# NKI-CCB/bcm3

Hardware: AMD Instinct MI355X
Metric: log-likelihood evals/sec (whole node), PopPK ODE @256 chains; HBM-roofline % (higher is better)
Workload: dtype f64

## Files before the change

### bcm3_amd/csrc/host/SamplerPTDevice.cpp

```cpp
#include "SamplerPTDevice.h"

#include <algorithm>
#include <cmath>
#include <condition_variable>
#include <cstring>
#include <deque>
#include <limits>
#include <map>
#include <mutex>
#include <thread>

#include "../../../include/bcm3.h"
#include "../../../include/bcm3hip.h"
#include "GMM.h"
#include "NetCDFClassic.h"
#include "log.h"

namespace bcm3 {

static const double kInf = std::numeric_limits<double>::infinity();


static uint64_t SplitMix64(uint64_t x)
{
// ... 151 lines not shown
    std::shared_ptr<LocalGroup> g_;
    int rank_;
};

}

std::unique_ptr<Transport> MakeLocalTransport(std::shared_ptr<LocalGroup> group, int rank)
{
    if (!group || rank < 0 || rank >= group->world) return nullptr;
    return std::unique_ptr<Transport>(new LocalTransport(std::move(group), rank));
}


namespace {

template <class T>
struct DevBuf {
    T* p = nullptr;
    size_t n = 0;
    bool alloc(size_t count)
    {
        n = count;
        return bcm3hip_malloc((void**)&p, std::max<size_t>(count, 1) * sizeof(T)) == 0;
    }
    ~DevBuf() { bcm3hip_free(p); }
};

template <class T>
bool Upload(DevBuf<T>& b, const std::vector<T>& h, void* s)
{
    return bcm3hip_memcpy_async(b.p, h.data(), h.size() * sizeof(T), BCM3HIP_H2D, s) == 0;
}
template <class T>
bool Download(std::vector<T>& h, const DevBuf<T>& b, void* s)
{
    h.resize(b.n);
    return bcm3hip_memcpy_async(h.data(), b.p, b.n * sizeof(T), BCM3HIP_D2H, s) == 0 && bcm3hip_stream_synchronize(s) == 0;
}

}

struct SamplerPTDevice::Impl {
    PTMHConfig cfg;
    std::shared_ptr<Likelihood> ll;
    std::unique_ptr<Transport> transport;
    void* stream = nullptr;
    bool own_stream = false;
    int64_t C = 0, Ctot = 0, g0 = 0;
    int d = 0, kmax = 1, H = 1, sub = 1;
    bool adaptive = true, adjusted = false;
    int kind = 1;
    std::vector<double> temps_host, prior_mean, prior_var;
    double target = 0.234;

    DevBuf<int32_t> pkind;
    DevBuf<double> p0, p1, p2, lower, upper, rw_scale, temps, zeros;
    DevBuf<double> values, prop, lprior, lprior_prop, llh, llh_prop, lpp, log_mh;
    DevBuf<int32_t> status, nan_flag;
    DevBuf<uint64_t> acc_mutate, acc_exchange;
    DevBuf<int32_t> ncomp, selected;
    DevBuf<double> weights, mean, chol, logc, scale, ema, work;
    bcm3hip_proposal P{};
    DevBuf<float> hist;
    DevBuf<int64_t> hcount;
    std::vector<std::unique_ptr<DevBuf<uint8_t>>> masks[2];
    bool mask_all[2] = {false, false};
    DevBuf<uint8_t> pair_mask;
    DevBuf<double> send_last, send_first, recv_next, recv_prev;

    PTMHCounters cnt;
    int64_t iter = 0, round = 0;

    bool blocked = false;
    int max_blocks = 1;
    std::vector<int32_t> bl_n, bl_off, bl_vars;
    std::vector<int64_t> sub_decisions;
    DevBuf<int32_t> b_nblocks, b_offset, b_vars, b_ncomp, b_selected;
    DevBuf<double> b_target, b_weights, b_logc, b_scale, b_ema, b_mean, b_chol;
    DevBuf<uint8_t> b_active;
    bcm3hip_blocks B{};

    bool spec_on = false;
    bool spec_tail_on = true;
    DevBuf<double> sp_cand_x, sp_cand_lp, sp_cand_lmh, sp_cand_llh, sp_cand_sc, sp_batch_x, sp_batch_llh;
    DevBuf<int32_t> sp_cand_sel, sp_cand_upd, sp_cand_steps, sp_steps_hint, sp_steps_prop, sp_batch_status,
        sp_batch_steps, sp_batch_src, sp_batch_n, sp_err;
    DevBuf<int32_t> sp_pos;
    DevBuf<float> sp_xs;
    DevBuf<int64_t> sp_total;
    DevBuf<uint8_t> sp_cand_active, acc_mut, acc_mut2, acc_exc;
    DevBuf<int32_t> partner[2], pair_first[2];
    DevBuf<double> sp_send_last, sp_send_first, sp_remote;
    DevBuf<uint8_t> cross_acc;
    DevBuf<int32_t> sp_pred;
    DevBuf<double> sp_inv_scale;
    bool cross_round[2] = {false, false};
    bcm3hip_spec S{};
    int64_t spec_pairs = 0;
    int spec_first_round = 0;

    std::unique_ptr<SampleFileWriter> out;
    DevBuf<double> out_buf;
    bool out_on = false, out_gather = false;
    DevBuf<double> out_recv;
    int64_t out_samples = 0, out_first = 0, out_pending = 0, emitted = 0;
    int out_flush = 64;
    bool out_overflow_logged = false;
    std::string adapt_file;
    BundleFile adapt_out;

    bool Emit()
    {
        const int64_t six = emitted++;
        if (!out_on) return true;
        if (six >= out_samples) {
            if (!out_overflow_logged) LOGWARNING("More samples than the output file holds (%lld); later samples are not stored", (long long)out_samples);
            out_overflow_logged = true;
            return true;
        }
        if (out_pending == 0) out_first = six;
        double* slot = out_buf.p + out_pending * C * (d + 2);
        if (bcm3hip_memcpy_async(slot, values.p, C * d * sizeof(double), BCM3HIP_D2D, stream) != 0 ||
            bcm3hip_memcpy_async(slot + C * d, lprior.p, C * sizeof(double), BCM3HIP_D2D, stream) != 0 ||
            bcm3hip_memcpy_async(slot + C * (d + 1), llh.p, C * sizeof(double), BCM3HIP_D2D, stream) != 0)
            return false;
        out_pending++;
        if (out_pending == out_flush || six + 1 == out_samples) return Flush();
        return true;
    }

    bool Flush()
    {
        if (!out_on || out_pending == 0) return true;
        if (out_gather) return FlushGather();
        std::vector<double> h((size_t)(out_pending * C * (d + 2)));
        if (bcm3hip_memcpy_async(h.data(), out_buf.p, h.size() * sizeof(double), BCM3HIP_D2H, stream) != 0 ||
            bcm3hip_stream_synchronize(stream) != 0)
            return false;
        const std::vector<double> w(C, 1.0);
        for (int64_t k = 0; k < out_pending; k++) {
            const double* r = &h[(size_t)(k * C * (d + 2))];
            if (!out->Write((size_t)(out_first + k), 0, (size_t)C, r, r + C * d, r + C * (d + 1), w.data())) {
                LOGERROR("Writing sample %lld to the output file failed", (long long)(out_first + k));
                return false;
            }
        }
        out_pending = 0;
        return true;
    }

    bool FlushGather()
    {
        const size_t cnt = (size_t)(out_pending * C * (d + 2));
        const int world = cfg.world, rank = cfg.rank;
        if (rank != 0) {
            const double* sp = out_buf.p;
            const int peer = 0;
            if (!transport || !transport->Exchange(1, &sp, &peer, 0, nullptr, nullptr, cnt, stream)) {
                LOGERROR("Sending sample rows to rank 0 failed (rank %d)", rank);
                return false;
            }
            out_pending = 0;
            return bcm3hip_stream_synchronize(stream) == 0;
        }
        std::vector<double*> recvs((size_t)(world - 1));
        std::vector<int> peers((size_t)(world - 1));
// ... 391 lines not shown
            speer[ns++] = Prev();
            recvs[nr] = recv_prev.p;
            rpeer[nr++] = Prev();
        }
        if (do_next) {
            recvs[nr] = recv_next.p;
            rpeer[nr++] = Next();
        }
        if (!transport || !transport->Exchange(ns, sends, speer, nr, recvs, rpeer, n, stream)) {
            LOGERROR("PT swap transport failed (rank %d)", cfg.rank);
            return false;
        }
        return Launch(bcm3hip_pt_cross_accept((int)C, d, g0, gp, do_next, do_prev, temps.p, values.p, llh.p,
                                              lprior.p, lpp.p, recv_next.p, recv_prev.p, acc_out,
                                              do_next ? acc_exchange.p : nullptr, cfg.seed, (uint64_t)round, stream),
                      "pt_cross_accept");
    }

    bool Exchange(uint8_t* acc_mask = nullptr, uint8_t* cross_out = nullptr)
    {
        if (Ctot < 2) return true;
        const int start = (int)(round % 2);
        const bool wrap_local = cfg.world == 1 && (Ctot - 1 - start) % 2 == 0;
        if (!Launch(bcm3hip_pt_exchange_local((int)C, d, g0, start, wrap_local ? 1 : 0, temps.p, values.p, llh.p,
                                              lprior.p, lpp.p, acc_mask, acc_exchange.p, cfg.seed, (uint64_t)round,
                                              stream),
                    "pt_exchange_local"))
            return false;
        int64_t attempted = wrap_local ? 1 : 0;
        for (int64_t i = 0; i + 1 < C; i++)
            if (((g0 + i - start) % 2 + 2) % 2 == 0) attempted++;
        if (cfg.world > 1 && ((g0 + C - 1 - start) % 2 + 2) % 2 == 0) {
            if (!Cross(true, true, (int64_t)Prev() * C + C - 1, cross_out)) return false;
            attempted++;
        }
        cnt.attempted_exchange += attempted;
        if (adaptive) {
            if (mask_all[start]) {
                if (!HistoryAdd(nullptr)) return false;
            } else {
                for (auto& m : masks[start])
                    if (!HistoryAdd(m->p)) return false;
            }
        }
        round++;
        return true;
    }

    bool ExchangeRandom()
    {
        const int64_t ci = RandomPair(cfg.seed, (uint64_t)round, Ctot);
        const int64_t l1 = ci - g0, l2 = ci + 1 - g0;
        if (0 <= l1 && l2 < C) {
            if (!Launch(bcm3hip_pt_exchange_pair((int)C, d, (int)l1, (int)l2, ci, temps.p, values.p, llh.p, lprior.p,
                                                 lpp.p, nullptr, acc_exchange.p, cfg.seed, (uint64_t)round, stream),
                        "pt_exchange_pair"))
                return false;
            cnt.attempted_exchange++;
        } else if (cfg.world > 1 && (l1 == C - 1 || l2 == 0)) {
            if (l1 == C - 1) {
                if (!Cross(true, false, 0)) return false;
                cnt.attempted_exchange++;
            } else if (!Cross(false, true, ci)) {
                return false;
            }
        }
        if (adaptive) {
            std::vector<uint8_t> m(C, 0);
            bool any = false;
            for (int64_t i : {l1, l2})
                if (0 <= i && i < C) {
                    m[i] = 1;
                    any = true;
                }
            if (any && (!Upload(pair_mask, m, stream) || !HistoryAdd(pair_mask.p))) return false;
        }
        round++;
        return true;
    }

    bool IterationOnce(bool last)
    {
        bool ok;
        if (Ctot < 2) {
            ok = Mutate();
        } else if (cfg.swapping_scheme == 0) {
            ok = Exchange();
            for (int s = 0; ok && s < cfg.exploration_steps; s++) ok = Mutate();
        } else if (MoveUniform(cfg.seed, (uint64_t)cnt.samples_done) < cfg.exchange_probability) {
            ok = (cfg.swapping_scheme == 1) ? Exchange() : ExchangeRandom();
        } else {
            ok = Mutate();
        }
        return ok && PostIteration(last);
    }

    bool AdaptDue(int64_t si, bool last) const
    {
        if (!adaptive || (si + 1) % cfg.use_every_nth != 0) return false;
        const int64_t sample_ix = si / cfg.use_every_nth;
        return cfg.adapt_proposal_samples > 0 && (sample_ix + 1) % cfg.adapt_proposal_samples == 0 && !last &&
               cnt.adaptations_done < cfg.adapt_proposal_times;
    }

    bool PostIteration(bool last)
    {
        const int64_t si = cnt.samples_done++;
        cnt.iterations++;
        if ((si + 1) % cfg.use_every_nth == 0 && !Emit()) return false;
        if (AdaptDue(si, last)) return Adapt();
        return true;
    }

    bool PairPossible() const { return spec_on && !AdaptDue(cnt.samples_done, false); }

    bool PairExchange()
    {
        const int st = (int)(round % 2);
        if (cfg.world == 1 && mask_all[st] && Ctot >= 2) {
            const bool wrap_local = (Ctot - 1 - st) % 2 == 0;
            int64_t attempted = wrap_local ? 1 : 0;
            for (int64_t i = 0; i + 1 < C; i++)
                if (((g0 + i - st) % 2 + 2) % 2 == 0) attempted++;
            if (!Launch(bcm3hip_ptmh_spec_exchange((int)C, d, g0, st, wrap_local ? 1 : 0, temps.p, values.p, llh.p,
                                                   lprior.p, lpp.p, acc_exc.p, acc_exchange.p, cfg.seed,
                                                   (uint64_t)round, partner[st].p, pair_first[st].p, &S, H, sub,
                                                   adaptive ? hist.p : nullptr, hcount.p, stream),
                        "ptmh_spec_exchange"))
                return false;
            cnt.attempted_exchange += attempted;
            round++;
            return true;
        }
        return Exchange(acc_exc.p, cross_acc.p) &&
               Launch(bcm3hip_ptmh_spec_track((int)C, nullptr, partner[st].p, pair_first[st].p, acc_exc.p, &S, stream),
                      "ptmh_spec_track");
    }

    bool TailFusable() const
    {
        const int st = (int)(round % 2);
        return cfg.world == 1 && mask_all[st] && Ctot >= 2 && C <= 4096 && S.batch_pos &&
               !(out_on && (cnt.samples_done + 1) % cfg.use_every_nth == 0) && spec_tail_on;
    }

    bool IterationPair(bool last)
    {
        if (!PairExchange()) return false;
        const int nxt = (int)(round % 2);
        if (!Launch(bcm3hip_ptmh_propose_adaptive((int)C, d, pkind.p, p0.p, p1.p, p2.p, temps.p, values.p, prop.p,
                                                  lprior_prop.p, log_mh.p, &P, g0, cfg.seed, (uint64_t)iter, stream),
                    "ptmh_propose_adaptive"))
            return false;
        if (cross_round[nxt]) {
            const size_t row = (size_t)d * sizeof(double);
            if (bcm3hip_memcpy_async(sp_send_last.p, values.p + (C - 1) * d, row, BCM3HIP_D2D, stream) != 0 ||
                bcm3hip_memcpy_async(sp_send_last.p + d, prop.p + (C - 1) * d, row, BCM3HIP_D2D, stream) != 0 ||
                bcm3hip_memcpy_async(sp_send_first.p, values.p, row, BCM3HIP_D2D, stream) != 0 ||
                bcm3hip_memcpy_async(sp_send_first.p + d, prop.p, row, BCM3HIP_D2D, stream) != 0)
                return false;
            const double* sends[2] = {sp_send_last.p, sp_send_first.p};
            const int speer[2] = {Next(), Prev()};
            double* recvs[2] = {sp_remote.p + 2 * d, sp_remote.p};
            const int rpeer[2] = {Prev(), Next()};
            if (!transport || !transport->Exchange(2, sends, speer, 2, recvs, rpeer, (size_t)(2 * d), stream)) {
                LOGERROR("speculative boundary rows: transport failed (rank %d)", cfg.rank);
                return false;
            }
        }
        if (!Launch(bcm3hip_ptmh_spec_candidates((int)C, d, pkind.p, p0.p, p1.p, p2.p, temps.p, values.p, prop.p,
                                                 partner[nxt].p, sp_remote.p, &P, &S, g0, cfg.seed, (uint64_t)iter + 1,
                                                 stream),
                    "ptmh_spec_candidates") ||
            !Launch(bcm3hip_ptmh_spec_batch((int)C, d, prop.p, partner[nxt].p, sp_inv_scale.p, spec_first_round, &S,
                                            stream),
                    "ptmh_spec_batch"))
            return false;
        cnt.likelihood_launches++;
        if (!ll->EvaluateLogProbabilityBatchDeviceCounted((size_t)C * (1 + BCM3HIP_SPEC_SLOTS), S.batch_n, S.batch_x,
                                                          S.batch_llh, S.batch_status, S.batch_steps, stream)) {
            LOGERROR("EvaluateLogProbabilityBatchDeviceCounted failed");
            return false;
        }
        if (TailFusable()) {
            const int st = (int)(round % 2);
            const bool wrap_local = (Ctot - 1 - st) % 2 == 0;
            int64_t attempted = wrap_local ? 1 : 0;
            for (int64_t i = 0; i + 1 < C; i++)
                if (((g0 + i - st) % 2 + 2) % 2 == 0) attempted++;
            if (!Launch(bcm3hip_ptmh_spec_tail((int)C, d, g0, st, wrap_local ? 1 : 0, temps.p, partner[st].p,
                                               pair_first[st].p, acc_mut.p, acc_mut2.p, acc_exc.p, cross_acc.p,
                                               sp_remote.p, acc_mutate.p, acc_exchange.p, &S, prop.p, lprior_prop.p,
                                               log_mh.p, llh_prop.p, cfg.learning_rate, values.p, lprior.p, llh.p, lpp.p,
                                               nan_flag.p, &P, cfg.seed, (uint64_t)iter, (uint64_t)round, H, sub, hist.p,
                                               hcount.p, sp_err.p, stream),
                        "ptmh_spec_tail"))
                return false;
            cnt.attempted_mutate += C;
            iter++;
            if (!PostIteration(false)) return false;
            cnt.attempted_exchange += attempted;
            round++;
            cnt.attempted_mutate += C;
            iter++;
            spec_pairs++;
            return PostIteration(last);
        }
        if (!Launch(bcm3hip_ptmh_spec_commit((int)C, d, 0, temps.p, nullptr, nullptr, nullptr, nullptr, nullptr, nullptr,
                                             &S, prop.p, lprior_prop.p, log_mh.p, llh_prop.p, cfg.learning_rate,
                                             values.p, lprior.p, llh.p, lpp.p, acc_mut.p, acc_mutate.p, nan_flag.p, &P,
                                             g0, cfg.seed, (uint64_t)iter, H, sub, hist.p, hcount.p, sp_err.p, stream),
                    "ptmh_spec_commit"))
            return false;
        cnt.attempted_mutate += C;
        iter++;
        if (!PostIteration(false)) return false;
        if (!PairExchange()) return false;
        if (!Launch(bcm3hip_ptmh_spec_commit((int)C, d, 1, temps.p, partner[nxt].p, pair_first[nxt].p, acc_mut.p,
                                             acc_exc.p, cross_acc.p, sp_remote.p, &S, prop.p, lprior_prop.p, log_mh.p,
                                             llh_prop.p, cfg.learning_rate, values.p, lprior.p, llh.p, lpp.p, acc_mut2.p,
                                             acc_mutate.p, nan_flag.p, &P, g0, cfg.seed, (uint64_t)iter, H, sub, hist.p,
                                             hcount.p, sp_err.p, stream),
                    "ptmh_spec_commit"))
            return false;
        cnt.attempted_mutate += C;
        iter++;
        spec_pairs++;
        return PostIteration(last);
    }

    bool Iterations(int64_t n, bool last_at_end, int64_t nan_every)
    {
        int64_t since_check = 0;
        for (int64_t i = 0; i < n;) {
            int64_t k;
            if (i + 2 <= n && PairPossible()) {
                if (!IterationPair(last_at_end && i + 2 == n)) return false;
                k = 2;
            } else {
                if (!IterationOnce(last_at_end && i + 1 == n)) return false;
                k = 1;
            }
            i += k;
            since_check += k;
            if (nan_every > 0 && since_check >= nan_every) {
                since_check = 0;
                if (!CheckNaN()) return false;
            }
        }
        return true;
    }

    bool SetupSpeculation()
    {
        spec_tail_on = getenv("BCM3_NO_SPEC_TAIL") == nullptr;
        spec_on = cfg.speculate != 0 && !blocked && adaptive && (cfg.world == 1 || transport) && cfg.swapping_scheme == 0 &&
                  cfg.exploration_steps == 1 && Ctot >= 2 && d <= 64 && C * (1 + BCM3HIP_SPEC_SLOTS) <= 4096 &&
                  ll->SupportsCountedBatch();
        if (!spec_on) return true;
        spec_first_round = bcm3hip_current_device_simds();
        const int64_t K = BCM3HIP_SPEC_SLOTS, N = C * (1 + K);
        bool ok = sp_cand_x.alloc(C * K * d) && sp_cand_lp.alloc(C * K) && sp_cand_lmh.alloc(C * K) &&
                  sp_cand_llh.alloc(C * K) && sp_cand_sc.alloc(C * K) && sp_cand_sel.alloc(C * K) &&
                  sp_cand_upd.alloc(C * K) && sp_cand_steps.alloc(C * K) && sp_cand_active.alloc(C * K) &&
                  sp_steps_hint.alloc(C) && sp_steps_prop.alloc(C) && sp_batch_x.alloc(N * d) &&
                  sp_batch_llh.alloc(N) && sp_batch_status.alloc(N) && sp_batch_steps.alloc(N) &&
                  sp_batch_src.alloc(N) && sp_batch_n.alloc(1) && sp_err.alloc(1) && acc_mut.alloc(C) &&
                  acc_mut2.alloc(C) &&
                  acc_exc.alloc(C) && sp_send_last.alloc(2 * d) && sp_send_first.alloc(2 * d) &&
                  sp_remote.alloc(4 * d) && cross_acc.alloc(2) && sp_pred.alloc(N) && sp_inv_scale.alloc(d) &&
                  sp_total.alloc(1) && sp_pos.alloc(N) && sp_xs.alloc(N * d);
        for (int st = 0; st < 2 && ok; st++) ok = partner[st].alloc(C) && pair_first[st].alloc(C);
        if (!ok) {
            LOGERROR("SamplerPTDevice: speculative buffers could not be allocated");
            return false;
        }
        for (int st = 0; st < 2; st++) {
            std::vector<int32_t> pa(C, -1), pf(C, -1);
            const int par = (int)(((g0 - st) % 2 + 2) % 2);
            for (int64_t i = par; i + 1 < C; i += 2) {
                pa[i] = (int32_t)(i + 1);
                pa[i + 1] = (int32_t)i;
                pf[i] = pf[i + 1] = (int32_t)i;
            }
            if (cfg.world == 1 && (Ctot - 1 - st) % 2 == 0) {
                pa[C - 1] = 0;
                pa[0] = (int32_t)(C - 1);
                pf[C - 1] = pf[0] = (int32_t)(C - 1);
            }
            cross_round[st] = cfg.world > 1 && ((g0 + C - 1 - st) % 2 + 2) % 2 == 0;
            if (cross_round[st]) {
                pa[C - 1] = BCM3HIP_SPEC_REMOTE_NEXT;
                pa[0] = BCM3HIP_SPEC_REMOTE_PREV;
            }
            if (!Upload(partner[st], pa, stream) || !Upload(pair_first[st], pf, stream)) return false;
        }
        std::vector<double> isc(d);
        for (int j = 0; j < d; j++)
            isc[j] = (prior_var[j] > 0.0 && std::isfinite(prior_var[j])) ? 1.0 / std::sqrt(prior_var[j]) : 1.0;
        if (!Upload(sp_inv_scale, isc, stream) ||
            bcm3hip_memset_async(sp_batch_n.p, 0, sizeof(int32_t), stream) != 0 ||
            bcm3hip_memset_async(sp_steps_hint.p, 0, C * sizeof(int32_t), stream) != 0 ||
            bcm3hip_memset_async(sp_batch_steps.p, 0, N * sizeof(int32_t), stream) != 0 ||
            bcm3hip_memset_async(sp_cand_steps.p, 0, C * K * sizeof(int32_t), stream) != 0 ||
            bcm3hip_memset_async(sp_err.p, 0, sizeof(int32_t), stream) != 0 ||
            bcm3hip_memset_async(sp_total.p, 0, sizeof(int64_t), stream) != 0)
            return false;
        S.cand_x = sp_cand_x.p;
        S.cand_lp = sp_cand_lp.p;
        S.cand_lmh = sp_cand_lmh.p;
        S.cand_llh = sp_cand_llh.p;
        S.cand_sel = sp_cand_sel.p;
        S.cand_upd = sp_cand_upd.p;
        S.cand_sc = sp_cand_sc.p;
        S.cand_active = sp_cand_active.p;
        S.cand_steps = sp_cand_steps.p;
        S.steps_hint = sp_steps_hint.p;
        S.steps_prop = sp_steps_prop.p;
        S.batch_x = sp_batch_x.p;
        S.batch_llh = sp_batch_llh.p;
        S.batch_status = sp_batch_status.p;
        S.batch_steps = sp_batch_steps.p;
        S.batch_src = sp_batch_src.p;
        S.batch_n = sp_batch_n.p;
        S.pred_steps = sp_pred.p;
        S.batch_total = sp_total.p;
        S.batch_pos = sp_pos.p;
        S.batch_xs = sp_xs.p;
        return true;
    }

    bool CheckNaN()
    {
        std::vector<int32_t> f;
        if (!Download(f, nan_flag, stream)) return false;
        if (f[0] != 0) {
            LOGERROR("Likelihood evaluation returned NaN (Sampler::EvaluateLikelihood, fatal)");
            return false;
// ... 461 lines not shown
```

### bcm3_amd/csrc/proposal_kernels.hip

```cpp
#include <hip/hip_runtime.h>

#include <cmath>
#include <cstdint>

#include "../../include/bcm3hip.h"
#include "ctr_rng.h"
#include "prior_marginal.h"
#include "pt_exchange.h"

namespace bcm3hip {
namespace {

using rng::normal01;
using rng::rng_key;
using rng::u01;

__device__ double logsum2(double loga, double logb)
{
    if (logb > loga) {
        const double t = loga;
        loga = logb;
        logb = t;
    }
    if (loga == -INFINITY) return loga;
// ... 1296 lines not shown
                                        bcm3hip_proposal P, int64_t chain0, uint64_t seed, uint64_t iter, int H,
                                        int subsampling, float* __restrict__ hist, int64_t* __restrict__ counters,
                                        int32_t* __restrict__ error)
{
    const int c = blockIdx.x * blockDim.x + threadIdx.x;
    if (c >= C) return;
    commit_one(c, C, d, select, temps, partner, pair_first, acc_prev, acc_exc, cross_acc, remote, S, prop, lprior_prop,
               log_mh, llh_prop, learning_rate, values, lprior, llh, lpp, acc_out, accepted, nan_llh, P, chain0, seed,
               iter, H, subsampling, hist, counters, error);
}

__global__ void ptmh_spec_track_accept_kernel(int C, const uint8_t* __restrict__ acc, bcm3hip_spec S)
{
    const int c = blockIdx.x * blockDim.x + threadIdx.x;
    if (c >= C) return;
    if (acc[c]) S.steps_hint[c] = S.steps_prop[c];
}
__global__ void __launch_bounds__(1024) ptmh_spec_track_exchange_kernel(int C, const int32_t* __restrict__ partner,
                                                                        const int32_t* __restrict__ pair_first,
                                                                        const uint8_t* __restrict__ acc_exc,
                                                                        bcm3hip_spec S)
{
    int v[4];
    int n = 0;
    for (int c = threadIdx.x; c < C && n < 4; c += blockDim.x, n++) {
        const int p = partner[c];
        v[n] = (p >= 0 && acc_exc[pair_first[c]]) ? S.steps_hint[p] : S.steps_hint[c];
    }
    __syncthreads();
    n = 0;
    for (int c = threadIdx.x; c < C && n < 4; c += blockDim.x, n++) S.steps_hint[c] = v[n];
}

__device__ __forceinline__ void exchange_round(int C, int d, int64_t g0, int start, int wrap_local, const double* temps, double* values,
                               double* llh, double* lprior, double* lpp, uint8_t* acc_mask,
                               unsigned long long* accepted, uint64_t seed, uint64_t round,
                               const int32_t* __restrict__ partner, const int32_t* __restrict__ pair_first,
                               const bcm3hip_spec& S, int H, int subsampling, float* __restrict__ hist,
                               int64_t* __restrict__ counters)
{
    const int par = (int)(((g0 - start) % 2 + 2) % 2);
    for (int p = threadIdx.x;; p += blockDim.x) {
        const int i = par + 2 * p;
        if (i + 1 >= C) break;
        exchange_pair(d, i, i + 1, g0 + i, temps, values, llh, lprior, lpp, acc_mask, accepted, seed, round);
    }
    __syncthreads();
    if (wrap_local && threadIdx.x == 0)
        exchange_pair(d, C - 1, 0, g0 + C - 1, temps, values, llh, lprior, lpp, acc_mask, accepted, seed, round);
    __syncthreads();
    int v[4];
    int n = 0;
    for (int c = threadIdx.x; c < C && n < 4; c += blockDim.x, n++) {
        const int p = partner[c];
        v[n] = (p >= 0 && acc_mask[pair_first[c]]) ? S.steps_hint[p] : S.steps_hint[c];
    }
    __syncthreads();
    n = 0;
    for (int c = threadIdx.x; c < C && n < 4; c += blockDim.x, n++) {
        S.steps_hint[c] = v[n];
        if (hist) history_one(c, d, H, subsampling, temps, values, nullptr, hist, counters);
    }
}

__global__ void __launch_bounds__(1024) ptmh_spec_exchange_kernel(
    int C, int d, int64_t g0, int start, int wrap_local, const double* temps, double* values, double* llh,
    double* lprior, double* lpp, uint8_t* acc_mask, unsigned long long* accepted, uint64_t seed, uint64_t round,
    const int32_t* __restrict__ partner, const int32_t* __restrict__ pair_first, bcm3hip_spec S, int H,
    int subsampling, float* __restrict__ hist, int64_t* __restrict__ counters)
{
    exchange_round(C, d, g0, start, wrap_local, temps, values, llh, lprior, lpp, acc_mask, accepted, seed, round, partner,
                   pair_first, S, H, subsampling, hist, counters);
}

__global__ void __launch_bounds__(1024) ptmh_spec_tail_kernel(
    int C, int d, int64_t g0, int start, int wrap_local, const double* __restrict__ temps,
    const int32_t* __restrict__ partner, const int32_t* __restrict__ pair_first, uint8_t* __restrict__ acc_mut,
    uint8_t* __restrict__ acc_mut2, uint8_t* __restrict__ acc_exc, const uint8_t* __restrict__ cross_acc,
    const double* __restrict__ remote, unsigned long long* __restrict__ acc_mutate,
    unsigned long long* __restrict__ acc_exchange, bcm3hip_spec S, double* __restrict__ prop,
    double* __restrict__ lprior_prop, double* __restrict__ log_mh, double* __restrict__ llh_prop, double learning_rate,
    double* __restrict__ values, double* __restrict__ lprior, double* __restrict__ llh, double* __restrict__ lpp,
    int32_t* __restrict__ nan_llh, bcm3hip_proposal P, uint64_t seed, uint64_t iter, uint64_t round, int H,
    int subsampling, float* __restrict__ hist, int64_t* __restrict__ counters, int32_t* __restrict__ error)
{
    for (int c = threadIdx.x; c < C; c += blockDim.x)
        commit_one(c, C, d, 0, temps, nullptr, nullptr, nullptr, nullptr, nullptr, nullptr, S, prop, lprior_prop, log_mh,
                   llh_prop, learning_rate, values, lprior, llh, lpp, acc_mut, acc_mutate, nan_llh, P, g0, seed, iter, H,
                   subsampling, hist, counters, error);
    __syncthreads();
    exchange_round(C, d, g0, start, wrap_local, temps, values, llh, lprior, lpp, acc_exc, acc_exchange, seed, round,
                   partner, pair_first, S, H, subsampling, hist, counters);
    __syncthreads();
    for (int c = threadIdx.x; c < C; c += blockDim.x)
        commit_one(c, C, d, 1, temps, partner, pair_first, acc_mut, acc_exc, cross_acc, remote, S, prop, lprior_prop,
                   log_mh, llh_prop, learning_rate, values, lprior, llh, lpp, acc_mut2, acc_mutate, nan_llh, P, g0, seed,
                   iter + 1, H, subsampling, hist, counters, error);
}

bool proposal_ok(const bcm3hip_proposal* P, int C, int d)
{
    if (!P || P->kmax < 1 || P->kmax > BCM3HIP_PROPOSAL_KMAX) return false;
    if (P->kind != BCM3HIP_PROPOSAL_GLOBAL_COVARIANCE && P->kind != BCM3HIP_PROPOSAL_GAUSSIAN_MIXTURE) return false;
    if (!(P->scaling_ema_period > 0.0) || !(P->t_dof >= 0.0)) return false;
    if (C > 0 && (!P->lower || !P->upper || !P->ncomp || !P->weights || !P->mean || !P->chol || !P->logc ||
                  !P->scale || !P->ema || !P->selected || !P->work))
        return false;
    return true;
}

}
}

using namespace bcm3hip;

extern "C" {

int bcm3hip_ptmh_propose_adaptive(int C, int d, const int32_t* prior_kind, const double* prior_p0,
                                  const double* prior_p1, const double* prior_p2, const double* temps,
                                  const double* values, double* prop, double* lprior_prop, double* log_mh,
                                  const bcm3hip_proposal* proposal, int64_t chain0, uint64_t seed, uint64_t iter,
                                  void* stream)
{
    if (C < 0 || d <= 0 || !proposal_ok(proposal, C, d) ||
        (C > 0 && (!prior_kind || !prior_p0 || !prior_p1 || !prior_p2 || !temps || !values || !prop ||
                   !lprior_prop || !log_mh)))
        return BCM3HIP_ERR_ARG;
    if (C == 0) return 0;
    if (d <= 64)
        hipLaunchKernelGGL(ptmh_propose_wave_kernel, dim3(C), dim3(64), 0, (hipStream_t)stream, C, d, prior_kind,
                           prior_p0, prior_p1, prior_p2, temps, values, prop, lprior_prop, log_mh, *proposal, chain0,
                           seed, iter);
    else
        hipLaunchKernelGGL(ptmh_propose_adaptive_kernel, dim3((C + 63) / 64), dim3(64), 0, (hipStream_t)stream, C,
                           d, prior_kind, prior_p0, prior_p1, prior_p2, temps, values, prop, lprior_prop, log_mh,
                           *proposal, chain0, seed, iter);
    return hipGetLastError() == hipSuccess ? 0 : BCM3HIP_ERR_HIP;
}

int bcm3hip_ptmh_accept_adaptive(int C, int d, const double* temps, const double* prop, const double* lprior_prop,
                                 const double* llh_prop, const double* log_mh, double learning_rate, double* values,
                                 double* lprior, double* llh, double* lpp, uint8_t* accept_out, uint64_t* accepted,
                                 int32_t* nan_llh, const bcm3hip_proposal* proposal, int64_t chain0, uint64_t seed,
                                 uint64_t iter, void* stream)
{
    if (C < 0 || d <= 0 || !proposal_ok(proposal, C, d) ||
        (C > 0 && (!temps || !prop || !lprior_prop || !llh_prop || !log_mh || !values || !lprior || !llh || !lpp)))
        return BCM3HIP_ERR_ARG;
    if (C == 0) return 0;
    hipLaunchKernelGGL(ptmh_accept_adaptive_kernel, dim3((C + 63) / 64), dim3(64), 0, (hipStream_t)stream, C, d,
                       temps, prop, lprior_prop, llh_prop, log_mh, learning_rate, values, lprior, llh, lpp, accept_out,
                       (unsigned long long*)accepted, nan_llh, *proposal, chain0, seed, iter);
    return hipGetLastError() == hipSuccess ? 0 : BCM3HIP_ERR_HIP;
}

static bool blocked_ok(const bcm3hip_proposal* P, const bcm3hip_blocks* B, int C, int d, int submove)
{
    if (!P || !B || d > BCM3HIP_BLOCKED_MAX_D || submove < 0 || submove >= d) return false;
    if (P->kind != BCM3HIP_PROPOSAL_GLOBAL_COVARIANCE && P->kind != BCM3HIP_PROPOSAL_GAUSSIAN_MIXTURE) return false;
    if (P->kmax < 1 || P->kmax > BCM3HIP_PROPOSAL_KMAX) return false;
    if (C > 0 && (!P->lower || !P->upper || !B->nblocks || !B->block_offset || !B->block_vars || !B->target ||
                  !B->ncomp || !B->selected || !B->weights || !B->logc || !B->scale || !B->ema || !B->mean ||
                  !B->chol || !B->active))
        return false;
    return true;
}

int bcm3hip_ptmh_propose_blocked(int C, int d, int submove, const int32_t* prior_kind, const double* prior_p0,
                                 const double* prior_p1, const double* prior_p2, const double* temps,
                                 const double* values, double* prop, double* lprior_prop, double* log_mh,
                                 const bcm3hip_proposal* proposal, const bcm3hip_blocks* blocks, int64_t chain0,
                                 uint64_t seed, uint64_t iter, void* stream)
{
    if (C < 0 || d <= 0 || !blocked_ok(proposal, blocks, C, d, submove) ||
        (C > 0 && (!prior_kind || !prior_p0 || !prior_p1 || !prior_p2 || !temps || !values || !prop ||
                   !lprior_prop || !log_mh)))
        return BCM3HIP_ERR_ARG;
    if (C == 0) return 0;
    if (d <= 64)
        hipLaunchKernelGGL(ptmh_propose_blocked_kernel, dim3(C), dim3(64), 0, (hipStream_t)stream, C, d, submove,
// ... 48 lines not shown

int bcm3hip_ptmh_spec_batch(int C, int d, const double* prop, const int32_t* partner, const double* inv_scale,
                            int first_round, const bcm3hip_spec* spec, void* stream)
{
    if (C <= 0 || d <= 0 || C * (1 + BCM3HIP_SPEC_SLOTS) > kSpecSortMax || !prop || !partner || !inv_scale ||
        first_round < 0 || !spec_ok(spec) || !spec->pred_steps)
        return BCM3HIP_ERR_ARG;
    hipLaunchKernelGGL(ptmh_spec_predict_kernel, dim3(C * (1 + BCM3HIP_SPEC_SLOTS)), dim3(64 * kKnnWaves), 0,
                       (hipStream_t)stream,
                       C, d, prop, partner, inv_scale, *spec);
    hipLaunchKernelGGL(ptmh_spec_batch_kernel, dim3(1), dim3(1024), 0, (hipStream_t)stream, C, d, prop, partner,
                       first_round, inv_scale, *spec);
    return hipGetLastError() == hipSuccess ? 0 : BCM3HIP_ERR_HIP;
}

int bcm3hip_ptmh_spec_scatter(int C, const bcm3hip_spec* spec, double* llh_prop, void* stream)
{
    if (C <= 0 || !spec_ok(spec) || !llh_prop) return BCM3HIP_ERR_ARG;
    const int n = C * (1 + BCM3HIP_SPEC_SLOTS);
    hipLaunchKernelGGL(ptmh_spec_scatter_kernel, dim3((n + 255) / 256), dim3(256), 0, (hipStream_t)stream, C, *spec,
                       llh_prop);
    return hipGetLastError() == hipSuccess ? 0 : BCM3HIP_ERR_HIP;
}

int bcm3hip_ptmh_spec_select(int C, int d, const double* temps, const int32_t* partner, const int32_t* pair_first,
                             const uint8_t* acc_mutate, const uint8_t* acc_exchange, const uint8_t* cross_acc,
                             const double* remote, const double* values, const bcm3hip_spec* spec, double* prop,
                             double* lprior_prop, double* log_mh, double* llh_prop, const bcm3hip_proposal* proposal,
                             int32_t* error, void* stream)
{
    if (C <= 0 || d <= 0 || !temps || !partner || !pair_first || !acc_mutate || !acc_exchange || !spec_ok(spec) ||
        !values || !prop || !lprior_prop || !log_mh || !llh_prop || !proposal_ok(proposal, C, d))
        return BCM3HIP_ERR_ARG;
    hipLaunchKernelGGL(ptmh_spec_select_kernel, dim3((C + 63) / 64), dim3(64), 0, (hipStream_t)stream, C, d, temps,
                       partner, pair_first, acc_mutate, acc_exchange, cross_acc, remote, values, *spec, prop,
                       lprior_prop, log_mh, llh_prop, *proposal, error);
    return hipGetLastError() == hipSuccess ? 0 : BCM3HIP_ERR_HIP;
}

int bcm3hip_ptmh_spec_commit(int C, int d, int select, const double* temps, const int32_t* partner,
                             const int32_t* pair_first, const uint8_t* acc_prev, const uint8_t* acc_exchange,
                             const uint8_t* cross_acc, const double* remote, const bcm3hip_spec* spec, double* prop,
                             double* lprior_prop, double* log_mh, double* llh_prop, double learning_rate, double* values,
                             double* lprior, double* llh, double* lpp, uint8_t* accept_out, uint64_t* accepted,
                             int32_t* nan_llh, const bcm3hip_proposal* proposal, int64_t chain0, uint64_t seed,
                             uint64_t iter, int H, int subsampling, float* history, int64_t* counters, int32_t* error,
                             void* stream)
{
    if (C <= 0 || d <= 0 || !spec_ok(spec) || !proposal_ok(proposal, C, d) || !temps || !prop || !lprior_prop ||
        !log_mh || !llh_prop || !values || !lprior || !llh || !lpp || !accept_out ||
        (select && (!partner || !pair_first || !acc_prev || !acc_exchange || acc_prev == accept_out)) ||
        (history && (H <= 0 || subsampling <= 0 || !counters)))
        return BCM3HIP_ERR_ARG;
    hipLaunchKernelGGL(ptmh_spec_commit_kernel, dim3((C + 63) / 64), dim3(64), 0, (hipStream_t)stream, C, d, select,
                       temps, partner, pair_first, acc_prev, acc_exchange, cross_acc, remote, *spec, prop, lprior_prop,
                       log_mh, llh_prop, learning_rate, values, lprior, llh, lpp, accept_out,
                       (unsigned long long*)accepted, nan_llh, *proposal, chain0, seed, iter, H, subsampling, history,
                       counters, error);
    return hipGetLastError() == hipSuccess ? 0 : BCM3HIP_ERR_HIP;
}

int bcm3hip_ptmh_spec_exchange(int C, int d, int64_t g0, int start, int wrap_local, const double* temps,
                               double* values, double* llh, double* lprior, double* lpp, uint8_t* acc_exchange,
                               uint64_t* accepted, uint64_t seed, uint64_t round, const int32_t* partner,
                               const int32_t* pair_first, const bcm3hip_spec* spec, int H, int subsampling,
                               float* history, int64_t* counters, void* stream)
{
    if (C < 2 || C > 4096 || d <= 0 || !temps || !values || !llh || !lprior || !lpp || !acc_exchange || !partner ||
        !pair_first || !spec_ok(spec) || (history && (H <= 0 || subsampling <= 0 || !counters)))
        return BCM3HIP_ERR_ARG;
    hipLaunchKernelGGL(ptmh_spec_exchange_kernel, dim3(1), dim3(1024), 0, (hipStream_t)stream, C, d, g0, start,
                       wrap_local, temps, values, llh, lprior, lpp, acc_exchange, (unsigned long long*)accepted, seed,
                       round, partner, pair_first, *spec, H, subsampling, history, counters);
    return hipGetLastError() == hipSuccess ? 0 : BCM3HIP_ERR_HIP;
}

int bcm3hip_ptmh_spec_tail(int C, int d, int64_t g0, int start, int wrap_local, const double* temps,
                           const int32_t* partner, const int32_t* pair_first, uint8_t* acc_mut, uint8_t* acc_mut2,
                           uint8_t* acc_exc, const uint8_t* cross_acc, const double* remote, uint64_t* accepted_mutate,
                           uint64_t* accepted_exchange, const bcm3hip_spec* spec, double* prop, double* lprior_prop,
                           double* log_mh, double* llh_prop, double learning_rate, double* values, double* lprior,
                           double* llh, double* lpp, int32_t* nan_llh, const bcm3hip_proposal* proposal, uint64_t seed,
                           uint64_t iter, uint64_t round, int H, int subsampling, float* history, int64_t* counters,
                           int32_t* error, void* stream)
{
    if (C < 2 || C > 4096 || d <= 0 || !spec_ok(spec) || !spec->batch_pos || !proposal_ok(proposal, C, d) || !temps ||
        !partner || !pair_first || !acc_mut || !acc_mut2 || acc_mut == acc_mut2 || !acc_exc || !prop || !lprior_prop ||
        !log_mh || !llh_prop || !values || !lprior || !llh || !lpp || (history && (H <= 0 || subsampling <= 0 || !counters)))
        return BCM3HIP_ERR_ARG;
    hipLaunchKernelGGL(ptmh_spec_tail_kernel, dim3(1), dim3(1024), 0, (hipStream_t)stream, C, d, g0, start, wrap_local,
                       temps, partner, pair_first, acc_mut, acc_mut2, acc_exc, cross_acc, remote,
                       (unsigned long long*)accepted_mutate, (unsigned long long*)accepted_exchange, *spec, prop,
                       lprior_prop, log_mh, llh_prop, learning_rate, values, lprior, llh, lpp, nan_llh, *proposal, seed,
                       iter, round, H, subsampling, history, counters, error);
    return hipGetLastError() == hipSuccess ? 0 : BCM3HIP_ERR_HIP;
}

int bcm3hip_ptmh_spec_track(int C, const uint8_t* acc_mutate, const int32_t* partner, const int32_t* pair_first,
                            const uint8_t* acc_exchange, const bcm3hip_spec* spec, void* stream)
{
    if (C <= 0 || C > 4096 || !spec_ok(spec) || (!acc_mutate && !acc_exchange) ||
        (acc_exchange && (!partner || !pair_first)))
        return BCM3HIP_ERR_ARG;
    if (acc_mutate)
        hipLaunchKernelGGL(ptmh_spec_track_accept_kernel, dim3((C + 255) / 256), dim3(256), 0, (hipStream_t)stream, C,
                           acc_mutate, *spec);
    else
        hipLaunchKernelGGL(ptmh_spec_track_exchange_kernel, dim3(1), dim3(1024), 0, (hipStream_t)stream, C, partner,
                           pair_first, acc_exchange, *spec);
    return hipGetLastError() == hipSuccess ? 0 : BCM3HIP_ERR_HIP;
}

int bcm3hip_gmm_eval(int n, int d, int K, const double* x, const double* mean, const double* chol, const double* logc,
                     const double* weights, double* logpdf, double* resp, void* stream)
{
    if (n < 0 || d <= 0 || d > 64 || K <= 0 || K > 64 || (n > 0 && (!x || !mean || !chol || !logc || !weights)))
        return BCM3HIP_ERR_ARG;
    if (n == 0) return 0;
    hipLaunchKernelGGL(gmm_eval_wave_kernel, dim3(n), dim3(64), 0, (hipStream_t)stream, n, d, K, x, mean, chol, logc,
                       weights, logpdf, resp);
    return hipGetLastError() == hipSuccess ? 0 : BCM3HIP_ERR_HIP;
}

int bcm3hip_history_add(int C, int d, int H, int subsampling, const double* temps, const double* values,
                        const uint8_t* mask, float* history, int64_t* counters, void* stream)
{
    if (C < 0 || d <= 0 || H <= 0 || subsampling <= 0 || (C > 0 && (!temps || !values || !history || !counters)))
        return BCM3HIP_ERR_ARG;
    if (C == 0) return 0;
    hipLaunchKernelGGL(history_add_kernel, dim3((C + 63) / 64), dim3(64), 0, (hipStream_t)stream, C, d, H,
                       subsampling, temps, values, mask, history, counters);
    return hipGetLastError() == hipSuccess ? 0 : BCM3HIP_ERR_HIP;
}

}
```

### include/bcm3hip.h

```cpp
#ifndef BCM3HIP_H
#define BCM3HIP_H

#if !defined(__HIPCC_RTC__)
#include <stddef.h>
#include <stdint.h>
#endif

#ifdef __cplusplus
extern "C" {
#endif

#define BCM3HIP_OK 0
#define BCM3HIP_ERR_ARG (-1)
#define BCM3HIP_ERR_HIP (-2)
#define BCM3HIP_ERR_NODEVICE (-3)
#define BCM3HIP_ERR_MODEL (-4)
#define BCM3HIP_ERR_ALLOC (-5)

#define BCM3HIP_STATUS_OK 0
#define BCM3HIP_STATUS_SOLVER_FAIL 1

enum {
    BCM3HIP_PK_ONE = 0,
    BCM3HIP_PK_TWO = 1,
// ... 356 lines not shown
    const int32_t* nblocks;
    const int32_t* block_offset;
    const int32_t* block_vars;
    const double* target;
    int32_t* ncomp;
    int32_t* selected;
    double* weights;
    double* logc;
    double* scale;
    double* ema;
    double* mean;
    double* chol;
    uint8_t* active;
} bcm3hip_blocks;
int bcm3hip_ptmh_propose_blocked(int C, int d, int submove, const int32_t* prior_kind, const double* prior_p0,
                                 const double* prior_p1, const double* prior_p2, const double* temps,
                                 const double* values, double* prop, double* lprior_prop, double* log_mh,
                                 const bcm3hip_proposal* proposal, const bcm3hip_blocks* blocks, int64_t chain0,
                                 uint64_t seed, uint64_t iter, void* stream);
int bcm3hip_ptmh_accept_blocked(int C, int d, int submove, const double* temps, const double* prop,
                                const double* lprior_prop, const double* llh_prop, const double* log_mh,
                                double learning_rate, double* values, double* lprior, double* llh, double* lpp,
                                uint8_t* accept_out, uint64_t* accepted, int32_t* nan_llh,
                                const bcm3hip_proposal* proposal, const bcm3hip_blocks* blocks, int64_t chain0,
                                uint64_t seed, uint64_t iter, void* stream);
enum { BCM3HIP_SPEC_SLOTS = 6 };
enum { BCM3HIP_SPEC_REMOTE_NEXT = -2, BCM3HIP_SPEC_REMOTE_PREV = -3 };
typedef struct {
    double* cand_x;
    double* cand_lp;
    double* cand_lmh;
    double* cand_llh;
    int32_t* cand_sel;
    int32_t* cand_upd;
    double* cand_sc;
    uint8_t* cand_active;
    int32_t* cand_steps;
    int32_t* steps_hint;
    int32_t* steps_prop;
    double* batch_x;
    double* batch_llh;
    int32_t* batch_status;
    int32_t* batch_steps;
    int32_t* batch_src;
    int32_t* batch_n;
    int32_t* pred_steps;
    int64_t* batch_total;
    int32_t* batch_pos;
    float* batch_xs;
} bcm3hip_spec;
int bcm3hip_ptmh_spec_candidates(int C, int d, const int32_t* prior_kind, const double* prior_p0,
                                 const double* prior_p1, const double* prior_p2, const double* temps,
                                 const double* values, const double* prop, const int32_t* partner,
                                 const double* remote, const bcm3hip_proposal* proposal, const bcm3hip_spec* spec,
                                 int64_t chain0, uint64_t seed, uint64_t iter_next, void* stream);
int bcm3hip_ptmh_spec_batch(int C, int d, const double* prop, const int32_t* partner, const double* inv_scale,
                            int first_round, const bcm3hip_spec* spec, void* stream);
int bcm3hip_ptmh_spec_scatter(int C, const bcm3hip_spec* spec, double* llh_prop, void* stream);
int bcm3hip_ptmh_spec_select(int C, int d, const double* temps, const int32_t* partner, const int32_t* pair_first,
                             const uint8_t* acc_mutate, const uint8_t* acc_exchange, const uint8_t* cross_acc,
                             const double* remote, const double* values, const bcm3hip_spec* spec, double* prop,
                             double* lprior_prop, double* log_mh, double* llh_prop, const bcm3hip_proposal* proposal,
                             int32_t* error, void* stream);
int bcm3hip_ptmh_spec_commit(int C, int d, int select, const double* temps, const int32_t* partner,
                             const int32_t* pair_first, const uint8_t* acc_prev, const uint8_t* acc_exchange,
                             const uint8_t* cross_acc, const double* remote, const bcm3hip_spec* spec, double* prop,
                             double* lprior_prop, double* log_mh, double* llh_prop, double learning_rate, double* values,
                             double* lprior, double* llh, double* lpp, uint8_t* accept_out, uint64_t* accepted,
                             int32_t* nan_llh, const bcm3hip_proposal* proposal, int64_t chain0, uint64_t seed,
                             uint64_t iter, int H, int subsampling, float* history, int64_t* counters, int32_t* error,
                             void* stream);
int bcm3hip_ptmh_spec_exchange(int C, int d, int64_t g0, int start, int wrap_local, const double* temps,
                               double* values, double* llh, double* lprior, double* lpp, uint8_t* acc_exchange,
                               uint64_t* accepted, uint64_t seed, uint64_t round, const int32_t* partner,
                               const int32_t* pair_first, const bcm3hip_spec* spec, int H, int subsampling,
                               float* history, int64_t* counters, void* stream);
int bcm3hip_ptmh_spec_tail(int C, int d, int64_t g0, int start, int wrap_local, const double* temps,
                           const int32_t* partner, const int32_t* pair_first, uint8_t* acc_mut, uint8_t* acc_mut2,
                           uint8_t* acc_exc, const uint8_t* cross_acc, const double* remote, uint64_t* accepted_mutate,
                           uint64_t* accepted_exchange, const bcm3hip_spec* spec, double* prop, double* lprior_prop,
                           double* log_mh, double* llh_prop, double learning_rate, double* values, double* lprior,
                           double* llh, double* lpp, int32_t* nan_llh, const bcm3hip_proposal* proposal, uint64_t seed,
                           uint64_t iter, uint64_t round, int H, int subsampling, float* history, int64_t* counters,
                           int32_t* error, void* stream);
int bcm3hip_ptmh_spec_track(int C, const uint8_t* acc_mutate, const int32_t* partner, const int32_t* pair_first,
                            const uint8_t* acc_exchange, const bcm3hip_spec* spec, void* stream);
int bcm3hip_gmm_eval(int n, int d, int K, const double* x, const double* mean, const double* chol, const double* logc,
                     const double* weights, double* logpdf, double* resp, void* stream);
int bcm3hip_history_add(int C, int d, int H, int subsampling, const double* temps, const double* values,
                        const uint8_t* mask, float* history, int64_t* counters, void* stream);

int bcm3hip_pt_exchange_pair(int C, int d, int i1, int i2, int64_t g1, const double* temps, double* values,
                             double* llh, double* lprior, double* lpp, uint8_t* acc_out, uint64_t* accepted,
                             uint64_t seed, uint64_t round, void* stream);

int bcm3hip_pt_pack_boundary(int C, int d, const double* temps, const double* values, const double* llh,
                             const double* lprior, const double* lpp, double* send_last, double* send_first,
                             void* stream);
int bcm3hip_pt_cross_accept(int C, int d, int64_t g0, int64_t gp, int do_next, int do_prev, const double* temps,
                            double* values, double* llh, double* lprior, double* lpp, const double* recv_next,
                            const double* recv_prev, uint8_t* acc_out, uint64_t* accepted, uint64_t seed,
                            uint64_t round, void* stream);

enum { BCM3HIP_H2D = 1, BCM3HIP_D2H = 2, BCM3HIP_D2D = 3 };
int bcm3hip_set_device(int device);
int bcm3hip_malloc(void** ptr, size_t bytes);
int bcm3hip_free(void* ptr);
int bcm3hip_memcpy_async(void* dst, const void* src, size_t bytes, int kind, void* stream);
int bcm3hip_memset_async(void* dst, int value, size_t bytes, void* stream);
int bcm3hip_stream_create(void** stream);
int bcm3hip_stream_destroy(void* stream);
int bcm3hip_stream_synchronize(void* stream);
#define BCM3HIP_NCCL_ID_BYTES 128
int bcm3hip_nccl_get_unique_id(void* id);
int bcm3hip_nccl_comm_init(const void* id, int rank, int world, void** comm);
int bcm3hip_nccl_comm_destroy(void* comm);
int bcm3hip_nccl_exchange(void* comm, int n_send, const double* const* send, const int* send_peer, int n_recv,
                          double* const* recv, const int* recv_peer, size_t count, void* stream);

int bcm3hip_eval_batch_detail(bcm3hip_ctx* ctx, size_t n, size_t d, const double* values, double* logp,
                              int32_t* status, double* patient_llh, double* traj, bcm3hip_traj_stats* stats);

#ifdef __cplusplus
}
#endif
#endif
```

Measured before the change: 254,400.

## Fold next exchange round into speculative tail kernel

```diff
diff --git a/bcm3_amd/csrc/host/SamplerPTDevice.cpp b/bcm3_amd/csrc/host/SamplerPTDevice.cpp
--- a/bcm3_amd/csrc/host/SamplerPTDevice.cpp
+++ b/bcm3_amd/csrc/host/SamplerPTDevice.cpp
@@ -257,6 +257,8 @@
 
     bool spec_on = false;
     bool spec_tail_on = true;
+    bool spec_fold_on = true;
+    bool exchange_ahead = false;
     DevBuf<double> sp_cand_x, sp_cand_lp, sp_cand_lmh, sp_cand_llh, sp_cand_sc, sp_batch_x, sp_batch_llh;
     DevBuf<int32_t> sp_cand_sel, sp_cand_upd, sp_cand_steps, sp_steps_hint, sp_steps_prop, sp_batch_status,
         sp_batch_steps, sp_batch_src, sp_batch_n, sp_err;
@@ -814,6 +816,10 @@
     bool IterationOnce(bool last)
     {
         bool ok;
+        if (exchange_ahead) {
+            LOGERROR("Speculative iteration: an exchange round ran ahead of a single iteration (internal error)");
+            return false;
+        }
         if (Ctot < 2) {
             ok = Mutate();
         } else if (cfg.swapping_scheme == 0) {
@@ -876,9 +882,20 @@
                !(out_on && (cnt.samples_done + 1) % cfg.use_every_nth == 0) && spec_tail_on;
     }
 
-    bool IterationPair(bool last)
-    {
-        if (!PairExchange()) return false;
+    bool ExchangeFoldable(bool last, bool more) const
+    {
+        const int64_t si = cnt.samples_done;
+        const int st2 = (int)((round + 1) % 2);
+        return spec_fold_on && more && !last && mask_all[st2] &&
+               !(out_on && (si + 2) % cfg.use_every_nth == 0) && !AdaptDue(si + 1, last) && !AdaptDue(si + 2, false);
+    }
+
+    bool IterationPair(bool last, bool more)
+    {
+        if (exchange_ahead)
+            exchange_ahead = false;
+        else if (!PairExchange())
+            return false;
         const int nxt = (int)(round % 2);
         if (!Launch(bcm3hip_ptmh_propose_adaptive((int)C, d, pkind.p, p0.p, p1.p, p2.p, temps.p, values.p, prop.p,
                                                   lprior_prop.p, log_mh.p, &P, g0, cfg.seed, (uint64_t)iter, stream),
@@ -920,12 +937,19 @@
             int64_t attempted = wrap_local ? 1 : 0;
             for (int64_t i = 0; i + 1 < C; i++)
                 if (((g0 + i - st) % 2 + 2) % 2 == 0) attempted++;
+            const bool fold = ExchangeFoldable(last, more);
+            const int st2 = 1 - st;
+            const bool wrap2 = (Ctot - 1 - st2) % 2 == 0;
+            int64_t attempted2 = wrap2 ? 1 : 0;
+            for (int64_t i = 0; i + 1 < C; i++)
+                if (((g0 + i - st2) % 2 + 2) % 2 == 0) attempted2++;
             if (!Launch(bcm3hip_ptmh_spec_tail((int)C, d, g0, st, wrap_local ? 1 : 0, temps.p, partner[st].p,
                                                pair_first[st].p, acc_mut.p, acc_mut2.p, acc_exc.p, cross_acc.p,
                                                sp_remote.p, acc_mutate.p, acc_exchange.p, &S, prop.p, lprior_prop.p,
                                                log_mh.p, llh_prop.p, cfg.learning_rate, values.p, lprior.p, llh.p, lpp.p,
                                                nan_flag.p, &P, cfg.seed, (uint64_t)iter, (uint64_t)round, H, sub, hist.p,
-                                               hcount.p, sp_err.p, stream),
+                                               hcount.p, sp_err.p, fold ? partner[st2].p : nullptr,
+                                               fold ? pair_first[st2].p : nullptr, wrap2 ? 1 : 0, stream),
                         "ptmh_spec_tail"))
                 return false;
             cnt.attempted_mutate += C;
@@ -936,7 +960,13 @@
             cnt.attempted_mutate += C;
             iter++;
             spec_pairs++;
-            return PostIteration(last);
+            if (!PostIteration(last)) return false;
+            if (fold) {
+                cnt.attempted_exchange += attempted2;
+                round++;
+                exchange_ahead = true;
+            }
+            return true;
         }
         if (!Launch(bcm3hip_ptmh_spec_commit((int)C, d, 0, temps.p, nullptr, nullptr, nullptr, nullptr, nullptr, nullptr,
                                              &S, prop.p, lprior_prop.p, log_mh.p, llh_prop.p, cfg.learning_rate,
@@ -967,7 +997,7 @@
         for (int64_t i = 0; i < n;) {
             int64_t k;
             if (i + 2 <= n && PairPossible()) {
-                if (!IterationPair(last_at_end && i + 2 == n)) return false;
+                if (!IterationPair(last_at_end && i + 2 == n, i + 4 <= n)) return false;
                 k = 2;
             } else {
                 if (!IterationOnce(last_at_end && i + 1 == n)) return false;
@@ -986,6 +1016,7 @@
     bool SetupSpeculation()
     {
         spec_tail_on = getenv("BCM3_NO_SPEC_TAIL") == nullptr;
+        spec_fold_on = getenv("BCM3_NO_SPEC_FOLD") == nullptr;
         spec_on = cfg.speculate != 0 && !blocked && adaptive && (cfg.world == 1 || transport) && cfg.swapping_scheme == 0 &&
                   cfg.exploration_steps == 1 && Ctot >= 2 && d <= 64 && C * (1 + BCM3HIP_SPEC_SLOTS) <= 4096 &&
                   ll->SupportsCountedBatch();
diff --git a/bcm3_amd/csrc/proposal_kernels.hip b/bcm3_amd/csrc/proposal_kernels.hip
--- a/bcm3_amd/csrc/proposal_kernels.hip
+++ b/bcm3_amd/csrc/proposal_kernels.hip
@@ -1402,7 +1402,8 @@
     double* __restrict__ lprior_prop, double* __restrict__ log_mh, double* __restrict__ llh_prop, double learning_rate,
     double* __restrict__ values, double* __restrict__ lprior, double* __restrict__ llh, double* __restrict__ lpp,
     int32_t* __restrict__ nan_llh, bcm3hip_proposal P, uint64_t seed, uint64_t iter, uint64_t round, int H,
-    int subsampling, float* __restrict__ hist, int64_t* __restrict__ counters, int32_t* __restrict__ error)
+    int subsampling, float* __restrict__ hist, int64_t* __restrict__ counters, int32_t* __restrict__ error,
+    const int32_t* __restrict__ partner_next, const int32_t* __restrict__ pair_first_next, int wrap_next)
 {
     for (int c = threadIdx.x; c < C; c += blockDim.x)
         commit_one(c, C, d, 0, temps, nullptr, nullptr, nullptr, nullptr, nullptr, nullptr, S, prop, lprior_prop, log_mh,
@@ -1416,6 +1417,11 @@
         commit_one(c, C, d, 1, temps, partner, pair_first, acc_mut, acc_exc, cross_acc, remote, S, prop, lprior_prop,
                    log_mh, llh_prop, learning_rate, values, lprior, llh, lpp, acc_mut2, acc_mutate, nan_llh, P, g0, seed,
                    iter + 1, H, subsampling, hist, counters, error);
+    if (partner_next) {
+        __syncthreads();
+        exchange_round(C, d, g0, 1 - start, wrap_next, temps, values, llh, lprior, lpp, acc_exc, acc_exchange, seed,
+                       round + 1, partner_next, pair_first_next, S, H, subsampling, hist, counters);
+    }
 }
 
 bool proposal_ok(const bcm3hip_proposal* P, int C, int d)
@@ -1630,17 +1636,19 @@
                            double* log_mh, double* llh_prop, double learning_rate, double* values, double* lprior,
                            double* llh, double* lpp, int32_t* nan_llh, const bcm3hip_proposal* proposal, uint64_t seed,
                            uint64_t iter, uint64_t round, int H, int subsampling, float* history, int64_t* counters,
-                           int32_t* error, void* stream)
+                           int32_t* error, const int32_t* partner_next, const int32_t* pair_first_next, int wrap_next,
+                           void* stream)
 {
     if (C < 2 || C > 4096 || d <= 0 || !spec_ok(spec) || !spec->batch_pos || !proposal_ok(proposal, C, d) || !temps ||
         !partner || !pair_first || !acc_mut || !acc_mut2 || acc_mut == acc_mut2 || !acc_exc || !prop || !lprior_prop ||
-        !log_mh || !llh_prop || !values || !lprior || !llh || !lpp || (history && (H <= 0 || subsampling <= 0 || !counters)))
+        !log_mh || !llh_prop || !values || !lprior || !llh || !lpp || (history && (H <= 0 || subsampling <= 0 || !counters)) ||
+        (start != 0 && start != 1) || (partner_next && !pair_first_next))
         return BCM3HIP_ERR_ARG;
     hipLaunchKernelGGL(ptmh_spec_tail_kernel, dim3(1), dim3(1024), 0, (hipStream_t)stream, C, d, g0, start, wrap_local,
                        temps, partner, pair_first, acc_mut, acc_mut2, acc_exc, cross_acc, remote,
                        (unsigned long long*)accepted_mutate, (unsigned long long*)accepted_exchange, *spec, prop,
                        lprior_prop, log_mh, llh_prop, learning_rate, values, lprior, llh, lpp, nan_llh, *proposal, seed,
-                       iter, round, H, subsampling, history, counters, error);
+                       iter, round, H, subsampling, history, counters, error, partner_next, pair_first_next, wrap_next);
     return hipGetLastError() == hipSuccess ? 0 : BCM3HIP_ERR_HIP;
 }
 
diff --git a/include/bcm3hip.h b/include/bcm3hip.h
--- a/include/bcm3hip.h
+++ b/include/bcm3hip.h
@@ -462,7 +462,8 @@
                            double* log_mh, double* llh_prop, double learning_rate, double* values, double* lprior,
                            double* llh, double* lpp, int32_t* nan_llh, const bcm3hip_proposal* proposal, uint64_t seed,
                            uint64_t iter, uint64_t round, int H, int subsampling, float* history, int64_t* counters,
-                           int32_t* error, void* stream);
+                           int32_t* error, const int32_t* partner_next, const int32_t* pair_first_next, int wrap_next,
+                           void* stream);
 int bcm3hip_ptmh_spec_track(int C, const uint8_t* acc_mutate, const int32_t* partner, const int32_t* pair_first,
                             const uint8_t* acc_exchange, const bcm3hip_spec* spec, void* stream);
 int bcm3hip_gmm_eval(int n, int d, int K, const double* x, const double* mean, const double* chol, const double* logc,
```

Result: no change. 253,600 (-0.3%).
